# teofum/yart

Measured on NVIDIA B200. Metric: Mrays/s at 1080p (primary + shadow rays, reference ray count), higher is better.
Workload: dtype f32

## Files before the change

include/yart_cuda.h:

```cpp
#ifndef YART_CUDA_H
#define YART_CUDA_H

#include <stddef.h>
#include <stdint.h>

#ifdef __cplusplus
extern "C" {
#endif

#define YC_OK 0
#define YC_ERR_INVALID (-1)
#define YC_ERR_CUDA (-2)
#define YC_ERR_NO_SCENE (-3)
#define YC_ERR_NO_DEVICE (-4)
#define YC_ERR_STATE (-5)
#define YC_ERR_IO (-6)
#define YC_ERR_UNSUPPORTED (-7)

#define YC_ERR_ABORTED (-8)

#define YC_MAX_NODE_DEPTH 16


typedef struct YcNode {
// ... 171 lines not shown

typedef struct YcStats {
  uint64_t raysReference;
  uint64_t raysExtend;
  uint64_t raysShadow;
  uint64_t samples;
  uint64_t kernelLaunches;
  double gpuMs;
  uint64_t boxTests, triTests;
  double extendMs;
  uint64_t extendLaunches;
  double shadeMs;
  uint64_t shadeLaunches;
  uint64_t hitsShaded;
  double commMs;
} YcStats;

typedef struct YcRay { float o[3], tmin, d[3], tmax; } YcRay;

typedef struct YcHit {
  float t;
  uint32_t prim;
  int32_t material;
  int32_t lightIdx;
  uint32_t backSide;
  uint32_t didHit;
  float p[3], n[3], tg[3], uv[2];
  float attenuation[3];
} YcHit;

// ... 169 lines not shown
```

yart_b200/capi.py:

```python
from __future__ import annotations

import ctypes as C
import os

HERE = os.path.dirname(os.path.abspath(__file__))
PRODUCT_LIB = os.path.join(HERE, "libyart_b200.so")
SAMPLERS_LIB = os.path.join(HERE, "libyart_b200_samplers.so")

YC_OK, YC_ERR_INVALID, YC_ERR_CUDA, YC_ERR_NO_SCENE, YC_ERR_NO_DEVICE, YC_ERR_STATE, YC_ERR_IO = 0, -1, -2, -3, -4, -5, -6
YC_ERR_UNSUPPORTED = -7
TONEMAP_NONE, TONEMAP_AGX, TONEMAP_AGX_GOLDEN, TONEMAP_AGX_PUNCHY = 0, 1, 2, 3
ESTIMATOR_GMON, ESTIMATOR_MON, ESTIMATOR_MEAN, ESTIMATOR_GMONB = 0, 1, 2, 3
TRACE_CLOSEST, TRACE_ANY, TRACE_COUNT, TRACE_USE_TMAX, TRACE_REFERENCE_ORDER, TRACE_WIDE = 0, 1, 16, 32, 64, 128

f32, u32, i32, u64 = C.c_float, C.c_uint32, C.c_int32, C.c_uint64


class YcCamera(C.Structure):
    _fields_ = [("position", f32 * 3), ("topLeftPixel", f32 * 3), ("pixelDeltaU", f32 * 3), ("pixelDeltaV", f32 * 3),
                ("frameX", f32 * 3), ("frameY", f32 * 3), ("frameZ", f32 * 3), ("apertureRadius", f32),
                ("apertureSides", u32), ("exposure", f32)]


BVH_SAH, BVH_MEDIAN_SPLIT, BVH_SAH_DEVICE, BVH_SAH_HOST = 0, 1, 2, 3
# ... 11 lines not shown


class YcRect(C.Structure):
    _fields_ = [("x", u32), ("y", u32), ("w", u32), ("h", u32)]


class YcFrameDesc(C.Structure):
    _fields_ = [("width", u32), ("height", u32), ("totalSamples", u32), ("tileSize", u32), ("background", f32 * 3),
                ("tonemap", u32), ("estimator", u32), ("shardIndex", u32), ("shardCount", u32)]


class YcStats(C.Structure):
    _fields_ = [("raysReference", u64), ("raysExtend", u64), ("raysShadow", u64), ("samples", u64),
                ("kernelLaunches", u64), ("gpuMs", C.c_double), ("boxTests", u64), ("triTests", u64),
                ("extendMs", C.c_double), ("extendLaunches", u64), ("shadeMs", C.c_double), ("shadeLaunches", u64),
                ("hitsShaded", u64), ("commMs", C.c_double)]


class YcRay(C.Structure):
    _fields_ = [("o", f32 * 3), ("tmin", f32), ("d", f32 * 3), ("tmax", f32)]


class YcHit(C.Structure):
    _fields_ = [("t", f32), ("prim", u32), ("material", i32), ("lightIdx", i32), ("backSide", u32), ("didHit", u32),
                ("p", f32 * 3), ("n", f32 * 3), ("tg", f32 * 3), ("uv", f32 * 2), ("attenuation", f32 * 3)]


class YcMesh(C.Structure):
    _fields_ = [("rootMin", f32 * 3), ("rootMax", f32 * 3), ("rootRef", u32), ("nodeOffset", u32), ("triOffset", u32),
                ("vertOffset", u32), ("primOffset", u32), ("nTris", u32), ("nVerts", u32), ("nInner", u32)]

# ... 146 lines not shown
```

yart_b200/csrc/integrator.cuh:

```cuda
#pragma once
#include "camera.cuh"
#include "lights.cuh"
#include "wide_bvh.cuh"

namespace yb {

constexpr uint32_t kFlagDepthMask = 0xffu;
constexpr uint32_t kFlagSpecular = 1u << 8;
constexpr uint32_t kFlagRegularized = 1u << 9;
constexpr uint32_t kFlagPendingRR = 1u << 10;
constexpr int32_t kHitMiss = -1;
constexpr int32_t kHitDead = -2;
constexpr uint32_t kBackSideBit = 1u << 30;

struct PathState {
  float4* rayO;
  float4* rayD;
  float4* L;
  float4* att;
  uint32_t* dim;
  uint32_t* flags;
  float4* hitA;
  int32_t* hitB;
};
// ... 98 lines not shown
  st.hit.prim = 0xffffffffu;
  st.hit.node = kHitMiss;
  st.hit.backSide = 0;
  st.attenuation = V3(1.0f);
}

template <bool ALPHA, bool COUNT, bool WIDE = false>
YB_DEV void extendStage(const DScene& sc, const WaveParams& w, const PathState& ps, uint32_t i, TravStack& stack,
                        TraceCounters& cnt) {
  static_assert(!(ALPHA && WIDE), "the wide walk does not reproduce the order of alpha-test sampler draws");
  V3 o, d;
  Sampler smp;
  if (!extendLoad<ALPHA>(w, ps, i, o, d, smp)) return;
  TraceState st;
  initTraceState(st, INFINITY);
  if (WIDE) traceSceneWide<false, COUNT, false>(sc, o, d, st, stack, cnt);
  else traceScene<false, ALPHA, COUNT, false>(sc, o, d, st, stack, &smp, cnt);
  extendStore<ALPHA>(ps, i, st, smp);
}

struct ShadowRequest {
  V3 o, d, lif, att;
  float tMax, absDotN, denom;
};

enum : uint32_t { kShadeContinue = 1u, kShadeShadow = 2u };

YB_DEV void shadeMissStage(const DScene& sc, const WaveParams& w, const PathState& ps, uint32_t i, uint32_t& raysReference) {
  raysReference += 1;
  const float4 ro4 = ps.rayO[i], rd4 = ps.rayD[i], L4 = ps.L[i], a4 = ps.att[i];
  const V3 rayD(rd4.x, rd4.y, rd4.z);
// ... 280 lines not shown
  V3 L(L4.x, L4.y, L4.z);
  L += V3(a4.x, a4.y, a4.z) * Ld;
  ps.L[i] = make_float4(L.x, L.y, L.z, 0.0f);
  return 1u;
}

template <bool ALPHA, bool COUNT, bool WIDE = false>
YB_DEV uint32_t shadowStage(const DScene& sc, const WaveParams& w, const PathState& ps, const ShadowQueue& q,
                            uint32_t j, TravStack& stack, TraceCounters& cnt) {
  V3 o, d;
  float tMax;
  Sampler smp;
  const uint32_t i = shadowLoad<ALPHA>(w, ps, q, j, o, d, tMax, smp);
  TraceState st;
  initTraceState(st, tMax);
  const bool occluded = WIDE ? traceSceneWide<true, COUNT, true>(sc, o, d, st, stack, cnt)
                             : traceScene<true, ALPHA, COUNT, !ALPHA>(sc, o, d, st, stack, &smp, cnt);
  return shadowFinish<ALPHA>(ps, q, j, i, st, occluded, smp);
}

}
```

yart_b200/csrc/trace_kernels.cuh:

```cuda
#pragma once
#include "integrator.cuh"

namespace yb {

constexpr int kTraceBlock = 128;

struct TraceTuning {
  int refillMin;
  int innerMin;
  int shEntries;
};

constexpr int kPsStack = kShStack + 1;
constexpr uint32_t kPsStride = kTraceBlock * 8;
constexpr int kSpillEntries = kMaxStack;
struct WarpStack {
  uint32_t base;
  uint32_t limit;
  uint2** spillBase;
  __device__ __forceinline__ void init(uint2* shStack, uint2** shSpill, uint2* spill, int shEntries) {
    base = uint32_t(__cvta_generic_to_shared(shStack + threadIdx.x));
    const uint32_t l = base + uint32_t(shEntries) * kPsStride;
    asm volatile("mov.u32 %0, %1;" : "=r"(limit) : "r"(l));
    if (threadIdx.x == 0) *shSpill = spill;
// ... 13 lines not shown
    }
    if (on) sa += kPsStride;
  }
  __device__ __forceinline__ void popIf(bool on, uint32_t& sa, uint32_t& ref, float& d) const {
    if (on) sa -= kPsStride;
    uint32_t x = ref, y = __float_as_uint(d);
    if (on && sa < limit) asm volatile("ld.shared.v2.u32 {%0, %1}, [%2];" : "=r"(x), "=r"(y) : "r"(sa));
    if (on && sa >= limit) {
      const uint2 v = *spillSlot(spillBase, sa - limit);
      x = v.x, y = v.y;
    }
    ref = x;
    d = __uint_as_float(y);
  }
  __device__ __forceinline__ void pop(uint32_t& sa, uint32_t& ref, float& d) const { popIf(true, sa, ref, d); }
};

__device__ __forceinline__ void nodeLocalRay(const DScene& sc, uint32_t node, int depth, V3& o, V3& d) {
  const int32_t* __restrict__ path = sc.nodePath + size_t(node) * YC_MAX_NODE_DEPTH;
#pragma unroll 1
  for (int level = 0; level <= depth; level++) {
    const YcNode& nd = sc.nodes[path[level]];
    const V3 no = xformRows(nd.inv, o, 1.0f), ndir = xformRows(nd.inv, d, 0.0f);
    o = no;
    d = ndir;
  }
}

struct NodeRec {
  float f[16];
// ... 187 lines not shown
```

yart_b200/csrc/trace_wide.cuh:

```cuda
#pragma once
#include "trace_kernels.cuh"

namespace yb {

struct Words8 {
  uint32_t w[8];
};
__device__ __forceinline__ Words8 loadHalfNode(const float4* p) {
  Words8 r;
  asm volatile("ld.global.nc.v8.b32 {%0,%1,%2,%3,%4,%5,%6,%7}, [%8];"
               : "=r"(r.w[0]), "=r"(r.w[1]), "=r"(r.w[2]), "=r"(r.w[3]), "=r"(r.w[4]), "=r"(r.w[5]), "=r"(r.w[6]), "=r"(r.w[7])
               : "l"(p));
  return r;
}

template <bool NEE, bool COUNT, class IO>
__device__ __forceinline__ void traceWidePersistent(const DScene& sc, IO& io, uint32_t n, uint32_t* head, uint2* spillBase,
                                                    const TraceTuning tune, TraceCounters& cnt) {
  __shared__ uint2 shStack[kPsStack * kTraceBlock];
  __shared__ uint2* shSpill;
  WarpStack stack;
  stack.init(shStack, &shSpill, spillBase, tune.shEntries);
  const unsigned FULL = 0xffffffffu;
  const unsigned lane = threadIdx.x & 31u, ltMask = (1u << lane) - 1u;

  int state = kLaneIdle;
  bool exhausted = false;
  uint32_t item = 0, nextNode = 0, cur = 0;
  uint32_t sp = 0;
  int curNode = 0;
  float dcur = 0.0f;
// ... 131 lines not shown
        } else {
          stack.pushIf(q0, sp, rf.x, t0);
          stack.pushIf(q1, sp, rf.y, t1);
          stack.pushIf(q2, sp, rf.z, t2);
          stack.pushIf(q3, sp, rf.w, t3);
        }
        cur = any ? nearRef : kPopRef;
        dcur = best;
      }
    }

    if (state == kLaneTrav && (int32_t(cur) < 0 || pend != 0u)) {
      {
        const uint32_t leaf = pend;
        const float leafD = pendD;
        if (int32_t(leaf) < -3 && leafD < st.hit.t && !(NEE && didHit)) {
          const YcMesh& mesh = sc.meshes[meshIdx];
          uint32_t ti = leaf & ~YC_REF_LEAF;
          while (true) {
            const float4 a = __ldg(tris + 3 * size_t(ti)), b = __ldg(tris + 3 * size_t(ti) + 1),
                         c = __ldg(tris + 3 * size_t(ti) + 2);
            meshHit |= testTriangle<NEE, false, COUNT>(sc, mesh, r, a, b, c, curNode, st, &smp, cnt);
            if (NEE && meshHit) break;
            if (__float_as_uint(c.z) & YC_TRI_LAST) break;
            ti++;
          }
          didHit |= meshHit;
        }
      }
      pend = 0u;
      if (NEE && didHit) {
        io.store(item, st, true, smp);
        state = kLaneIdle;
      } else if (cur == kNoRef) {
        state = kLaneNode;
      }
    }
  }
}

}
```

yart_b200/csrc/wavefront.cu:

```cuda
#include <algorithm>
#include <cstdarg>
#include <vector>

#include "estimator.cuh"
#include "integrator.cuh"
#include "rt.cuh"
#include "comm.cuh"
#include "bvh_build.cuh"
#ifndef YB_HOSTSIM
#include "trace_wide.cuh"
#endif

using namespace yb;

#ifndef YB_TRACE_MIN_BLOCKS
#define YB_TRACE_MIN_BLOCKS 7
#endif
#ifndef YB_SHADOW_MIN_BLOCKS
#define YB_SHADOW_MIN_BLOCKS 7
#endif
#ifndef YB_RESOLVE_MIN_BLOCKS
#define YB_RESOLVE_MIN_BLOCKS 4
#endif
#ifndef YB_SAMPLE_MIN_BLOCKS
// ... 55 lines not shown
  size_t bucketCapacity = 0;
  bool bucketsDirty = false;

  uint32_t* dCtr = nullptr;
  void* dSpill = nullptr;
  Counters* dCounters = nullptr;
  std::vector<void*> waveAllocs;

  rt::Event ev0, ev1;
  bool wavesPending = false;
  rt::Event evFinal;
  std::vector<std::pair<rt::Event, rt::Event>> extendEvents;
  size_t extendEventsUsed = 0;
  std::vector<std::pair<rt::Event, rt::Event>> shadeEvents;
  size_t shadeEventsUsed = 0;
  double shadeMs = 0, commMs = 0;
  uint64_t shadeLaunches = 0, hitsShaded = 0;
  bool timeShade = false;
  bool oneLane = false;
  uint64_t launches = 0;
  double gpuMs = 0, extendMs = 0;
  uint64_t extendLaunches = 0, raysExtend = 0;
  bool timeExtend = false, countTraversal = false;
  uint32_t tailThreshold = 16384;
  const volatile int32_t* abortFlag = nullptr;
  std::unique_ptr<Comm> comm;
  bool wide = false;
  int wideDepth = 0;
  uint64_t nWideNodes = 0;
};

static int settleWaves(yc_ctx* ctx);

// ... 323 lines not shown
  if (COUNT) {
    aggregatedCount(&counters->boxTests, cnt.box);
    aggregatedCount(&counters->triTests, cnt.tri);
  }
}

#ifndef YB_WIDE_MIN_BLOCKS
#define YB_WIDE_MIN_BLOCKS 7
#endif
template <bool COUNT>
__global__ void __launch_bounds__(kTraceBlock, YB_WIDE_MIN_BLOCKS) extendWideKernel(DScene sc, WaveParams w, PathState ps, const uint32_t* queue,
                                                              uint32_t n, uint32_t* ctr, Counters* counters, uint2* spill,
                                                              TraceTuning tune) {
  ExtendIO<false> io{w, ps, queue};
  TraceCounters cnt;
  traceWidePersistent<false, COUNT>(sc, io, n, ctr + kCtrExtendHead, spill, tune, cnt);
  if (COUNT) {
    aggregatedCount(&counters->boxTests, cnt.box);
    aggregatedCount(&counters->triTests, cnt.tri);
  }
}

template <bool COUNT>
__global__ void __launch_bounds__(kTraceBlock, YB_WIDE_MIN_BLOCKS) shadowWideKernel(DScene sc, WaveParams w, PathState ps, ShadowQueue sq,
                                                              uint32_t* ctr, Counters* counters, uint2* spill, TraceTuning tune) {
  const uint32_t n = ctr[kCtrShadowCount];
  ShadowIO<false> io{w, ps, sq};
  TraceCounters cnt;
  traceWidePersistent<true, COUNT>(sc, io, n, ctr + kCtrShadowHead, spill, tune, cnt);
  aggregatedCount(&counters->raysReference, io.contributed);
  if (blockIdx.x == 0 && threadIdx.x == 0) atomicAdd(&counters->raysShadow, (unsigned long long)n);
  if (COUNT) {
    aggregatedCount(&counters->boxTests, cnt.box);
    aggregatedCount(&counters->triTests, cnt.tri);
  }
}

constexpr int kTailBlock = 128;
struct TailGatherK {
  PathState ps, ts;
  const uint32_t* queue;
  uint32_t* tq;
  YB_DEV void operator()(uint32_t j) const {
    const uint32_t i = queue[j];
// ... 89 lines not shown
      rt::eventCreate(ctx->extendEvents.back().second);
    }
    ev = &ctx->extendEvents[ctx->extendEventsUsed++];
    rt::eventRecord(L.st, ev->first);
  }
  if (!ALPHA && !COUNT && ctx->wide)
    extendWideKernel<false><<<traceGrid(ctx, n), kTraceBlock, 0, L.st.s>>>(ctx->ds, L.w, L.ps, L.qA, n, L.ctr, ctx->dCounters,
                                                                           static_cast<uint2*>(L.spill), tuning(ctx));
  else
    extendKernel<ALPHA, COUNT><<<traceGrid(ctx, n), kTraceBlock, 0, L.st.s>>>(ctx->ds, L.w, L.ps, L.qA, n, L.ctr, ctx->dCounters,
                                                                              static_cast<uint2*>(L.spill), tuning(ctx));
  if (ev) rt::eventRecord(L.st, ev->second);
}
template <bool ALPHA, bool COUNT>
static void runShadow(yc_ctx* ctx, Lane& L, uint32_t upperBound) {
  if (!ALPHA && !COUNT && ctx->wide)
    shadowWideKernel<false><<<traceGrid(ctx, upperBound), kTraceBlock, 0, L.st.s>>>(
      ctx->ds, L.w, L.ps, L.sq, L.ctr, ctx->dCounters, static_cast<uint2*>(L.spill), tuning(ctx));
  else
    shadowKernel<ALPHA, COUNT><<<traceGrid(ctx, upperBound), kTraceBlock, 0, L.st.s>>>(
      ctx->ds, L.w, L.ps, L.sq, L.ctr, ctx->dCounters, static_cast<uint2*>(L.spill), tuning(ctx));
}
#endif

extern "C" int yc_create(int device, const YcOptions* opts, yc_ctx** out) {
  if (!out) return YC_ERR_INVALID;
  *out = nullptr;
  yc_ctx* ctx = new (std::nothrow) yc_ctx();
  if (!ctx) return YC_ERR_INVALID;
  if (opts) ctx->opts = *opts;
  if (ctx->opts.maxDepth == 0) ctx->opts.maxDepth = 30;
  if (ctx->opts.integrator > YC_INTEGRATOR_NAIVE || ctx->opts.scrambler > YC_SCRAMBLER_BINARY_PERMUTE ||
      ctx->opts.sampler > YC_SAMPLER_STRATIFIED || ctx->opts.lightSampler > YC_LIGHT_SAMPLER_UNIFORM ||
      ctx->opts.traversal > YC_TRAVERSAL_WIDE ||
      (ctx->opts.integrator == YC_INTEGRATOR_NAIVE && ctx->opts.maxDepth + 1 > kNaiveMaxSegments)) {
    delete ctx;
// ... 54 lines not shown

static void destroyComm(yc_ctx* ctx);
static void detachCombinedFrames(yc_ctx* ctx);

extern "C" void yc_destroy(yc_ctx* ctx) {
  if (!ctx) return;
  enter(ctx);
  rt::sync(ctx->st);
  destroyComm(ctx);
  freeFrame(ctx);
  freeAll(ctx->sceneAllocs);
  freeAll(ctx->waveAllocs);
  rt::eventDestroy(ctx->ev0);
  rt::eventDestroy(ctx->ev1);
  rt::eventDestroy(ctx->evFinal);
  for (auto* evs : {&ctx->extendEvents, &ctx->shadeEvents})
    for (auto& ev : *evs) {
      rt::eventDestroy(ev.first);
      rt::eventDestroy(ev.second);
    }
  for (int l = 0; l < kLanes; l++) {
    Lane& L = ctx->lanes[l];
    rt::sync(L.st);
    rt::sync(L.side);
    rt::hostRelease(L.hCtr);
    rt::eventDestroy(L.evCtr);
    rt::eventDestroy(L.evChunk);
    rt::eventDestroy(L.evTail);
    rt::eventDestroy(L.evSide[0]);
    rt::eventDestroy(L.evSide[1]);
    rt::destroy(L.side);
// ... 246 lines not shown
      return fail(ctx, YC_ERR_CUDA, "yc_begin_frame: %s", e);
    }
    ctx->bucketsDirty = true;
  }
  ctx->frame = *f;
  ctx->frame.shardCount = shardCount;
  if (ctx->bucketsDirty) {
    YC_TRY(rt::zero(ctx->st, ctx->dBuckets, ctx->bucketCapacity * kMaxBuckets * sizeof(float4)));
    ctx->bucketsDirty = false;
  }
  YC_TRY(rt::zero(ctx->st, ctx->dHdr, frameTexels * sizeof(float4)));
  YC_TRY(rt::zero(ctx->st, ctx->dLdr, frameTexels * sizeof(float4)));
  YC_TRY(rt::zero(ctx->st, ctx->dCounters, sizeof(Counters)));
  YC_TRY(rt::sync(ctx->st));
  ctx->launches = 0;
  ctx->gpuMs = ctx->extendMs = ctx->shadeMs = ctx->commMs = 0;
  ctx->extendLaunches = ctx->shadeLaunches = ctx->hitsShaded = 0;
  ctx->raysExtend = 0;
  ctx->inFrame = true;
  return YC_OK;
}

template <bool ALPHA>
static int issueBounce(yc_ctx* ctx, Lane& L) {
  const uint32_t n = L.n;
  YC_TRY(rt::zero(L.st, L.ctr, kCtrCount * sizeof(uint32_t)));
  if (ctx->countTraversal) runExtend<ALPHA, true>(ctx, L, n);
  else runExtend<ALPHA, false>(ctx, L, n);
  rt::launchFor(L.st, n, SortMissK{ctx->ds, L.w, L.ps, L.qA, L.qH, L.ctr, ctx->dCounters});
  std::pair<rt::Event, rt::Event>* sev = nullptr;
  if (ctx->timeShade) {
    if (ctx->shadeEventsUsed == ctx->shadeEvents.size()) {
// ... 256 lines not shown
    YC_TRY(rt::sync(ctx->lanes[l].st));
    YC_TRY(rt::sync(ctx->lanes[l].side));
  }
  YC_TRY(rt::lastError());
  ctx->gpuMs += rt::eventElapsedMs(ctx->ev0, ctx->ev1);
  for (size_t i = 0; i < ctx->extendEventsUsed; i++) {
    ctx->extendMs += rt::eventElapsedMs(ctx->extendEvents[i].first, ctx->extendEvents[i].second);
    ctx->extendLaunches++;
  }
  ctx->extendEventsUsed = 0;
  for (size_t i = 0; i < ctx->shadeEventsUsed; i++) {
    ctx->shadeMs += rt::eventElapsedMs(ctx->shadeEvents[i].first, ctx->shadeEvents[i].second);
    ctx->shadeLaunches++;
  }
  ctx->shadeEventsUsed = 0;
  return YC_OK;
}

static int accumulateWave(yc_ctx* ctx, const uint32_t* dList, uint32_t nPixCall, uint32_t sampleOffset, uint32_t waveSamples,
                          uint32_t bucketShard, uint32_t bucketShardCount) {
  const uint32_t m = waveBuckets(ctx->frame, waveSamples);
  ctx->bucketsDirty = true;
  return ctx->ds.hasAlpha ? renderChunks<true>(ctx, dList, nPixCall, sampleOffset, waveSamples, m, bucketShard, bucketShardCount)
                          : renderChunks<false>(ctx, dList, nPixCall, sampleOffset, waveSamples, m, bucketShard, bucketShardCount);
}

static void finalizeWave(yc_ctx* ctx, const uint32_t* dList, uint32_t nPixCall, uint32_t waveSamples, uint32_t takenBefore) {
  const YcFrameDesc& f = ctx->frame;
  const uint32_t takenAfter = takenBefore + waveSamples;
  const float wCurrent = float(takenBefore) / float(takenAfter), wWave = float(waveSamples) / float(takenAfter);
// ... 113 lines not shown
  if (!stats) return YC_OK;
  Counters c{};
  if (ctx->dCounters) YC_TRY(rt::d2h(ctx->st, &c, ctx->dCounters, sizeof c));
  memset(stats, 0, sizeof *stats);
  stats->raysReference = c.raysReference;
  stats->raysExtend = ctx->raysExtend + c.raysExtend;
  stats->raysShadow = c.raysShadow;
  stats->boxTests = c.boxTests;
  stats->triTests = c.triTests;
  stats->kernelLaunches = ctx->launches;
  stats->gpuMs = ctx->gpuMs;
  stats->extendMs = ctx->extendMs;
  stats->shadeMs = ctx->shadeMs, stats->shadeLaunches = ctx->shadeLaunches, stats->hitsShaded = ctx->hitsShaded;
  stats->commMs = ctx->commMs;
  stats->extendLaunches = ctx->extendLaunches;
  return YC_OK;
}

extern "C" int yc_resolve(yc_ctx* ctx, float* hdrRGBA, float* ldrRGBA, YcStats* stats) {
  if (!ctx) return YC_ERR_INVALID;
  YC_ENTER(ctx);
  if (!ctx->inFrame) return fail(ctx, YC_ERR_STATE, "yc_resolve before yc_begin_frame");
  const size_t bytes = size_t(ctx->frame.width) * ctx->frame.height * sizeof(float4);
  if (hdrRGBA) YC_TRY(rt::d2h(ctx->st, hdrRGBA, ctx->dHdr, bytes));
  if (ldrRGBA) YC_TRY(rt::d2h(ctx->st, ldrRGBA, ctx->dLdr, bytes));
  return readStats(ctx, stats);
}

extern "C" int yc_frame_device_ptrs(yc_ctx* ctx, void** hdr, void** ldr, size_t* bytes) {
  if (!ctx) return YC_ERR_INVALID;
// ... 11 lines not shown
  if (!ctx->inFrame) return fail(ctx, YC_ERR_STATE, "no frame");
  rt::launchFor(ctx->st, ctx->frame.width * ctx->frame.height, RetonemapK{ctx->dHdr, ctx->dLdr, ctx->frame.tonemap});
  ctx->launches++;
  YC_TRY(rt::sync(ctx->st));
  YC_TRY(rt::lastError());
  return YC_OK;
}

extern "C" int yc_set_profiling(yc_ctx* ctx, int timeExtendKernel) {
  if (!ctx) return YC_ERR_INVALID;
  YC_ENTER(ctx);
  ctx->timeExtend = (timeExtendKernel & 1) != 0;
  ctx->countTraversal = (timeExtendKernel & 2) != 0;
  ctx->timeShade = (timeExtendKernel & 4) != 0;
  ctx->oneLane = (timeExtendKernel & 8) != 0;
  return YC_OK;
}

YB_DEV Sampler traceHookSampler() {
  SamplerConfig c;
  c.log2spp = 4;
  c.nBase4Digits = 6 + 2;
  c.scrambler = kScrambleFastOwen;
  c.kind = kSamplerSobol;
  c.strata = 4;
  Sampler s;
  s.start(c, 0, 0, 0);
  return s;
}

template <bool NEE, bool ALPHA, bool COUNT, bool WIDE = false>
YB_DEV void traceOne(const DScene& sc, const YcRay& ray, bool useTMax, YcHit& out, TravStack& stack, TraceCounters& cnt) {
  Sampler smp = traceHookSampler();
  TraceState st;
  st.hit.t = (NEE || useTMax) ? ray.tmax : INFINITY;
  st.hit.node = kHitMiss;
  st.hit.u = st.hit.v = 0.0f;
  st.hit.prim = 0xffffffffu;
  st.hit.backSide = 0;
  st.attenuation = V3(1.0f);
  const V3 o(ray.o), d(ray.d);
  const bool did = WIDE ? traceSceneWide<NEE, COUNT, NEE>(sc, o, d, st, stack, cnt)
                        : traceScene<NEE, ALPHA, COUNT, false>(sc, o, d, st, stack, &smp, cnt);
  out.t = st.hit.t;
  out.didHit = did ? 1u : 0u;
  out.prim = did ? st.hit.prim : 0xffffffffu;
  out.material = -1, out.lightIdx = -1, out.backSide = 0;
  for (int k = 0; k < 3; k++) out.p[k] = out.n[k] = out.tg[k] = 0.0f;
  out.uv[0] = out.uv[1] = 0.0f;
  out.attenuation[0] = st.attenuation.x, out.attenuation[1] = st.attenuation.y, out.attenuation[2] = st.attenuation.z;
  if (did) {
    const SurfaceHit s = resolveHit(sc, st.hit, o, d);
    out.material = s.material, out.lightIdx = s.lightIdx, out.backSide = st.hit.backSide;
    out.p[0] = s.p.x, out.p[1] = s.p.y, out.p[2] = s.p.z;
    out.n[0] = s.n.x, out.n[1] = s.n.y, out.n[2] = s.n.z;
    out.tg[0] = s.tg.x, out.tg[1] = s.tg.y, out.tg[2] = s.tg.z;
    out.uv[0] = s.uv.x, out.uv[1] = s.uv.y;
// ... 74 lines not shown
  TraceIO<NEE, ALPHA, COMPACT> io{sc, rays, hits, compact, useTMax};
  TraceCounters cnt;
  tracePersistent<NEE, ALPHA, COUNT, false>(sc, io, n, head, spill, tune, cnt);
  if (COUNT) {
    aggregatedCount(&counters->boxTests, cnt.box);
    aggregatedCount(&counters->triTests, cnt.tri);
  }
}

template <bool NEE, bool COUNT, bool COMPACT>
__global__ void __launch_bounds__(kTraceBlock, YB_WIDE_MIN_BLOCKS) traceWideKernel(DScene sc, const YcRay* rays, uint32_t n, int useTMax, YcHit* hits,
                                                             CompactHit* compact, uint32_t* head, Counters* counters,
                                                             uint2* spill, TraceTuning tune) {
  TraceIO<NEE, false, COMPACT> io{sc, rays, hits, compact, useTMax};
  TraceCounters cnt;
  traceWidePersistent<NEE, COUNT>(sc, io, n, head, spill, tune, cnt);
  if (COUNT) {
    aggregatedCount(&counters->boxTests, cnt.box);
    aggregatedCount(&counters->triTests, cnt.tri);
  }
}

template <bool NEE, bool ALPHA, bool COUNT, bool WIDE = false>
static void runTrace(yc_ctx* ctx, const YcRay* rays, uint32_t n, bool useTMax, YcHit* hits, CompactHit* compact) {
  const int grid = traceGrid(ctx, n);
  uint2* spill = static_cast<uint2*>(ctx->dSpill);
  if (WIDE) {
    if (compact)
      traceWideKernel<NEE, COUNT, true><<<grid, kTraceBlock, 0, ctx->st.s>>>(ctx->ds, rays, n, useTMax, hits, compact, ctx->dCtr,
                                                                             ctx->dCounters, spill, tuning(ctx));
    else
// ... 587 lines not shown
```

yart_b200/csrc/wide_bvh.cuh:

```cuda
#pragma once
#include <vector>

#include "traverse.cuh"

#include <atomic>
#include <chrono>
#include <cstdio>
#include <cstdlib>
#include <thread>

namespace yb {

constexpr uint32_t kWideEmpty = 0xfffffffdu;

struct WideNode {
  float pS[3];
  float S[3];
  uint32_t q[6];
  uint32_t ref[4];
};
static_assert(sizeof(WideNode) == 64, "WideNode is two 32-byte sectors");

struct WideChildBox {
  float lo[3], hi[3];
// ... 212 lines not shown
  return tn <= tf;
}

template <int K>
YB_DEV float planeUnit(uint32_t word, uint32_t one) {
#ifdef YB_HOSTSIM
  return __uint_as_float(__byte_perm(word, one, 0x7604u | (uint32_t(K) << 4)));
#else
  uint32_t r;
  asm("prmt.b32 %0, %1, %2, %3;" : "=r"(r) : "r"(word), "r"(one), "n"(0x7604 | (K << 4)));
  return __uint_as_float(r);
#endif
}

struct WideSlabs {
  float tn[4];
  bool hit[4];
};
template <int K>
YB_DEV void slabWideChild(WideSlabs& r, uint32_t one, uint32_t nx, uint32_t ny, uint32_t nz, uint32_t fx, uint32_t fy, uint32_t fz,
                          float Sx, float Sy, float Sz, float Bx, float By, float Bz, float tmn, float tmx, bool live) {
  const float tnx = fmaExact(planeUnit<K>(nx, one), Sx, Bx), tny = fmaExact(planeUnit<K>(ny, one), Sy, By),
              tnz = fmaExact(planeUnit<K>(nz, one), Sz, Bz);
  const float tfx = fmaExact(planeUnit<K>(fx, one), Sx, Bx), tfy = fmaExact(planeUnit<K>(fy, one), Sy, By),
              tfz = fmaExact(planeUnit<K>(fz, one), Sz, Bz);
  r.tn[K] = fmaxf(fmaxf(tnx, tny), fmaxf(tnz, tmn));
  const float tf = fminf(fminf(tfx, tfy), fminf(tfz, tmx));
  r.hit[K] = live && r.tn[K] <= tf;
}
YB_DEV WideSlabs slabWide4(const WideRay& w, uint32_t one, float px, float py, float pz, float sx, float sy, float sz, uint32_t qlx,
                           uint32_t qhx, uint32_t qly, uint32_t qhy, uint32_t qlz, uint32_t qhz, float tmn, float tmx, bool live) {
  const float Sx = sx * w.idir.x, Sy = sy * w.idir.y, Sz = sz * w.idir.z;
  const float Bx = fmaExact(px, w.idir.x, w.odir.x), By = fmaExact(py, w.idir.y, w.odir.y), Bz = fmaExact(pz, w.idir.z, w.odir.z);
  const uint32_t nx = (qlx & ~w.mx) | (qhx & w.mx), fx = (qhx & ~w.mx) | (qlx & w.mx);
  const uint32_t ny = (qly & ~w.my) | (qhy & w.my), fy = (qhy & ~w.my) | (qly & w.my);
  const uint32_t nz = (qlz & ~w.mz) | (qhz & w.mz), fz = (qhz & ~w.mz) | (qlz & w.mz);
  WideSlabs r;
  slabWideChild<0>(r, one, nx, ny, nz, fx, fy, fz, Sx, Sy, Sz, Bx, By, Bz, tmn, tmx, live);
  slabWideChild<1>(r, one, nx, ny, nz, fx, fy, fz, Sx, Sy, Sz, Bx, By, Bz, tmn, tmx, live);
  slabWideChild<2>(r, one, nx, ny, nz, fx, fy, fz, Sx, Sy, Sz, Bx, By, Bz, tmn, tmx, live);
  slabWideChild<3>(r, one, nx, ny, nz, fx, fy, fz, Sx, Sy, Sz, Bx, By, Bz, tmn, tmx, live);
  return r;
}

template <bool NEE, bool COUNT, bool EARLY_OUT>
YB_DEV bool testBVHWide(const DScene& sc, const YcMesh& mesh, const WideMesh& wm, const LocalRay& r, const WideRay& w,
                        int nodeIdx, TraceState& st, TravStack& stack, TraceCounters& cnt) {
  float d;
  if (COUNT) cnt.box++;
  if (!slabWideBox(w, V3(mesh.rootMin), V3(mesh.rootMax), kTMin, st.hit.t, d)) return false;
  const float4* __restrict__ nodes = sc.wideNodes + 4 * size_t(wm.nodeOffset);
  const float4* __restrict__ tris = sc.bvhTris + 3 * size_t(mesh.triOffset);
  uint32_t cur = wm.rootRef;
  int sp = 0;
  bool didHit = false;
  while (true) {
    if (d < st.hit.t) {
      if (cur & YC_REF_LEAF) {
        uint32_t ti = cur & ~YC_REF_LEAF;
        while (true) {
          const float4 a = __ldg(tris + 3 * size_t(ti)), b = __ldg(tris + 3 * size_t(ti) + 1),
                       c = __ldg(tris + 3 * size_t(ti) + 2);
          didHit |= testTriangle<NEE, false, COUNT>(sc, mesh, r, a, b, c, nodeIdx, st, nullptr, cnt);
          if (NEE && didHit) break;
          if (__float_as_uint(c.z) & YC_TRI_LAST) break;
          ti++;
        }
        if (NEE && EARLY_OUT && didHit) return true;
        if (sp == 0) break;
        stack.pop(--sp, cur, d);
      } else {
        const float4* n = nodes + 4 * size_t(cur);
        const float4 r0 = __ldg(n), r1 = __ldg(n + 1), r2 = __ldg(n + 2), rf = __ldg(n + 3);
        const uint32_t ref[4] = {__float_as_uint(rf.x), __float_as_uint(rf.y), __float_as_uint(rf.z), __float_as_uint(rf.w)};
        WideSlabs sl = slabWide4(w, 0x3f800000u, r0.x, r0.y, r0.z, r0.w, r1.x, r1.y, __float_as_uint(r1.z), __float_as_uint(r1.w),
                                 __float_as_uint(r2.x), __float_as_uint(r2.y), __float_as_uint(r2.z), __float_as_uint(r2.w), kTMin,
                                 st.hit.t, true);
        float* tn = sl.tn;
        bool* hit = sl.hit;
        hit[2] = hit[2] && ref[2] != kWideEmpty;
        hit[3] = hit[3] && ref[3] != kWideEmpty;
        if (COUNT) cnt.box += 2u + (ref[2] != kWideEmpty) + (ref[3] != kWideEmpty);
        int nearSlot = -1;
// ... 5 lines not shown
        } else {
          for (int k = 0; k < 4; k++)
            if (hit[k] && k != nearSlot) stack.push(sp++, ref[k], tn[k]);
          cur = ref[nearSlot];
          d = tn[nearSlot];
        }
      }
    } else {
      if (sp == 0) break;
      stack.pop(--sp, cur, d);
    }
  }
  return didHit;
}

template <bool NEE, bool COUNT, bool EARLY_OUT>
YB_DEV bool traceSceneWide(const DScene& sc, V3 origin, V3 dir, TraceState& st, TravStack& stack, TraceCounters& cnt) {
  V3 ro[YC_MAX_NODE_DEPTH + 1], rd[YC_MAX_NODE_DEPTH + 1];
  ro[0] = origin;
  rd[0] = dir;
  bool didHit = false;
  uint32_t i = 0;
  while (i < sc.nNodes) {
    const YcNode& nd = sc.nodes[i];
    const int k = nd.depth;
    LocalRay r;
    r.o = xformRows(nd.inv, ro[k], 1.0f), r.d = xformRows(nd.inv, rd[k], 0.0f);
    ro[k + 1] = r.o;
    rd[k + 1] = r.d;
    WideRay w;
    w.set(r.o, r.d);
    float d;
    if (COUNT) cnt.box++;
    if (!slabWideBox(w, V3(nd.bmin), V3(nd.bmax), kTMin, st.hit.t, d) || st.hit.t < d) {
      i = uint32_t(nd.skip);
      continue;
    }
    if (nd.mesh >= 0) {
      const bool h = testBVHWide<NEE, COUNT, EARLY_OUT>(sc, sc.meshes[nd.mesh], sc.wideMeshes[nd.mesh], r, w, int(i), st, stack, cnt);
      didHit |= h;
      if (NEE && EARLY_OUT && h) return true;
    }
    i++;
  }
  return didHit;
}

}
```

yart_b200/host/api.cpp:

```cpp
#include <atomic>
#include <chrono>
#include <mutex>
#include <new>
#include <thread>
#include <cstring>
#include <vector>

#include "scene.hpp"

using namespace yartb;

namespace yartb {
bool loadGlb(const std::string& path, ysc::SceneDesc& out, std::string* err);
bool writePpm(const std::string& path, const float* rgba, uint32_t w, uint32_t h);
bool decodeTextureForTest(const uint8_t* png, size_t len, uint32_t type, int C, const int* channels, ysc::TextureDesc& out,
                          std::string& err);
bool decodeRadianceHdr(const uint8_t* data, size_t len, int& w, int& h, std::vector<float>& rgb, std::string& err);
}

struct ys_scene {
  HostScene host;
};

static thread_local std::string g_ysError;
// ... 568 lines not shown
  return writePpm(path, ldr.data(), r->s.width, r->s.height) ? YC_OK : rfail(r, YC_ERR_IO, std::string("cannot write ") + path);
}

extern "C" int yr_read(yr_renderer* r, float* hdrRGBA, float* ldrRGBA, YcStats* stats) {
  if (!r) return YC_ERR_INVALID;
  int rc = readFrames(r, hdrRGBA, ldrRGBA);
  if (rc != YC_OK) return rfail(r, rc, yc_last_error(r->shards[0].ctx));
  if (stats) {
    memset(stats, 0, sizeof *stats);
    for (Shard& sh : r->shards) {
      YcStats st{};
      if ((rc = yc_resolve(sh.ctx, nullptr, nullptr, &st)) != YC_OK) return rfail(r, rc, yc_last_error(sh.ctx));
      stats->raysReference += st.raysReference, stats->raysExtend += st.raysExtend, stats->raysShadow += st.raysShadow;
      stats->kernelLaunches += st.kernelLaunches, stats->boxTests += st.boxTests, stats->triTests += st.triTests;
      stats->gpuMs = std::max(stats->gpuMs, st.gpuMs), stats->extendMs += st.extendMs, stats->extendLaunches += st.extendLaunches;
    }
  }
  return YC_OK;
}

extern "C" const float* ys_lut_tables(size_t* count) {
  static HostScene holder;
  static std::once_flag once;
  std::call_once(once, [] {
    std::string err;
    holder.loadLuts(&err);
  });
  if (count) *count = holder.lutTables.size();
  return holder.lutTables.empty() ? nullptr : holder.lutTables.data();
}
// ... 1 lines not shown
```

Before: 1073.

## Add dedicated any-hit wide BVH traversal for shadow rays with ref-only stack

Splits shadow/any-hit traversal out of the closest-hit persistent wide BVH walker into its own kernel path. The new path keeps a 32-bit ref-only shared stack with no distances, and orders children by slab overlap length instead of entry distance so likely occluders are visited first. It also returns on the first triangle hit. The aim is to cut shared-memory traffic, register pressure and wasted node visits for occlusion rays. In exchange it adds code duplication plus some shadow-kernel timing instrumentation, and the child-ordering heuristic may not pay off on every scene.

```diff
diff --git a/include/yart_cuda.h b/include/yart_cuda.h
--- a/include/yart_cuda.h
+++ b/include/yart_cuda.h
@@ -209,6 +209,8 @@
   uint64_t shadeLaunches;
   uint64_t hitsShaded;
   double commMs;
+  double shadowMs;
+  uint64_t shadowLaunches;
 } YcStats;
 
 typedef struct YcRay { float o[3], tmin, d[3], tmax; } YcRay;
diff --git a/yart_b200/capi.py b/yart_b200/capi.py
--- a/yart_b200/capi.py
+++ b/yart_b200/capi.py
@@ -49,7 +49,7 @@
     _fields_ = [("raysReference", u64), ("raysExtend", u64), ("raysShadow", u64), ("samples", u64),
                 ("kernelLaunches", u64), ("gpuMs", C.c_double), ("boxTests", u64), ("triTests", u64),
                 ("extendMs", C.c_double), ("extendLaunches", u64), ("shadeMs", C.c_double), ("shadeLaunches", u64),
-                ("hitsShaded", u64), ("commMs", C.c_double)]
+                ("hitsShaded", u64), ("commMs", C.c_double), ("shadowMs", C.c_double), ("shadowLaunches", u64)]
 
 
 class YcRay(C.Structure):
diff --git a/yart_b200/csrc/integrator.cuh b/yart_b200/csrc/integrator.cuh
--- a/yart_b200/csrc/integrator.cuh
+++ b/yart_b200/csrc/integrator.cuh
@@ -136,7 +136,7 @@
   if (!extendLoad<ALPHA>(w, ps, i, o, d, smp)) return;
   TraceState st;
   initTraceState(st, INFINITY);
-  if (WIDE) traceSceneWide<false, COUNT, false>(sc, o, d, st, stack, cnt);
+  if (WIDE) traceSceneWide<false, COUNT>(sc, o, d, st, stack, cnt);
   else traceScene<false, ALPHA, COUNT, false>(sc, o, d, st, stack, &smp, cnt);
   extendStore<ALPHA>(ps, i, st, smp);
 }
@@ -447,7 +447,7 @@
   const uint32_t i = shadowLoad<ALPHA>(w, ps, q, j, o, d, tMax, smp);
   TraceState st;
   initTraceState(st, tMax);
-  const bool occluded = WIDE ? traceSceneWide<true, COUNT, true>(sc, o, d, st, stack, cnt)
+  const bool occluded = WIDE ? traceSceneWide<true, COUNT>(sc, o, d, st, stack, cnt)
                              : traceScene<true, ALPHA, COUNT, !ALPHA>(sc, o, d, st, stack, &smp, cnt);
   return shadowFinish<ALPHA>(ps, q, j, i, st, occluded, smp);
 }
diff --git a/yart_b200/csrc/trace_kernels.cuh b/yart_b200/csrc/trace_kernels.cuh
--- a/yart_b200/csrc/trace_kernels.cuh
+++ b/yart_b200/csrc/trace_kernels.cuh
@@ -51,6 +51,38 @@
     d = __uint_as_float(y);
   }
   __device__ __forceinline__ void pop(uint32_t& sa, uint32_t& ref, float& d) const { popIf(true, sa, ref, d); }
+};
+
+constexpr uint32_t kRsStride = kTraceBlock * 4;
+struct WarpRefStack {
+  uint32_t base, limit;
+  uint2** spillBase;
+  __device__ __forceinline__ void init(uint32_t* shStack, uint2** shSpill, uint2* spill, int shEntries) {
+    base = uint32_t(__cvta_generic_to_shared(shStack + threadIdx.x));
+    const uint32_t l = base + uint32_t(shEntries) * kRsStride;
+    asm volatile("mov.u32 %0, %1;" : "=r"(limit) : "r"(l));
+    if (threadIdx.x == 0) *shSpill = spill;
+    __syncthreads();
+    spillBase = shSpill;
+  }
+  __device__ __noinline__ static uint32_t* spillSlot(uint2** spillBase, uint32_t off) {
+    return reinterpret_cast<uint32_t*>(*spillBase + size_t(blockIdx.x * kTraceBlock + threadIdx.x) * kSpillEntries) + off / kRsStride;
+  }
+  __device__ __forceinline__ void put(uint32_t sa, uint32_t ref) const { asm volatile("st.shared.u32 [%0], %1;" ::"r"(sa), "r"(ref)); }
+  __device__ __forceinline__ void pushIf(bool on, uint32_t& sa, uint32_t ref) const {
+    if (on && sa < limit) put(sa, ref);
+    if (on && sa >= limit) {
+      if (sa < base + uint32_t(kMaxStack + 1) * kRsStride) *spillSlot(spillBase, sa - limit) = ref;
+    }
+    if (on) sa += kRsStride;
+  }
+  __device__ __forceinline__ void popIf(bool on, uint32_t& sa, uint32_t& ref) const {
+    if (on) sa -= kRsStride;
+    uint32_t x = ref;
+    if (on && sa < limit) asm volatile("ld.shared.u32 %0, [%1];" : "=r"(x) : "r"(sa));
+    if (on && sa >= limit) x = *spillSlot(spillBase, sa - limit);
+    ref = x;
+  }
 };
 
 __device__ __forceinline__ void nodeLocalRay(const DScene& sc, uint32_t node, int depth, V3& o, V3& d) {
diff --git a/yart_b200/csrc/trace_wide.cuh b/yart_b200/csrc/trace_wide.cuh
--- a/yart_b200/csrc/trace_wide.cuh
+++ b/yart_b200/csrc/trace_wide.cuh
@@ -14,7 +14,7 @@
   return r;
 }
 
-template <bool NEE, bool COUNT, class IO>
+template <bool COUNT, class IO>
 __device__ __forceinline__ void traceWidePersistent(const DScene& sc, IO& io, uint32_t n, uint32_t* head, uint2* spillBase,
                                                     const TraceTuning tune, TraceCounters& cnt) {
   __shared__ uint2 shStack[kPsStack * kTraceBlock];
@@ -176,14 +176,13 @@
       {
         const uint32_t leaf = pend;
         const float leafD = pendD;
-        if (int32_t(leaf) < -3 && leafD < st.hit.t && !(NEE && didHit)) {
+        if (int32_t(leaf) < -3 && leafD < st.hit.t) {
           const YcMesh& mesh = sc.meshes[meshIdx];
           uint32_t ti = leaf & ~YC_REF_LEAF;
           while (true) {
             const float4 a = __ldg(tris + 3 * size_t(ti)), b = __ldg(tris + 3 * size_t(ti) + 1),
                          c = __ldg(tris + 3 * size_t(ti) + 2);
-            meshHit |= testTriangle<NEE, false, COUNT>(sc, mesh, r, a, b, c, curNode, st, &smp, cnt);
-            if (NEE && meshHit) break;
+            meshHit |= testTriangle<false, false, COUNT>(sc, mesh, r, a, b, c, curNode, st, &smp, cnt);
             if (__float_as_uint(c.z) & YC_TRI_LAST) break;
             ti++;
           }
@@ -191,7 +190,175 @@
         }
       }
       pend = 0u;
-      if (NEE && didHit) {
+      if (cur == kNoRef) state = kLaneNode;
+    }
+  }
+}
+
+template <bool COUNT, class IO>
+__device__ __forceinline__ void anyHitWidePersistent(const DScene& sc, IO& io, uint32_t n, uint32_t* head, uint2* spillBase,
+                                                     const TraceTuning tune, TraceCounters& cnt) {
+  __shared__ uint32_t shStack[kPsStack * kTraceBlock];
+  __shared__ uint2* shSpill;
+  WarpRefStack stack;
+  stack.init(shStack, &shSpill, spillBase, tune.shEntries);
+  const unsigned FULL = 0xffffffffu;
+  const unsigned lane = threadIdx.x & 31u, ltMask = (1u << lane) - 1u;
+
+  int state = kLaneIdle;
+  bool exhausted = false;
+  uint32_t item = 0, nextNode = 0, cur = 0;
+  uint32_t sp = 0;
+  int curNode = 0;
+  bool rayIsWorld = false, worldFinite = false;
+  V3 wo, wd;
+  LocalRay r;
+  WideRay wr;
+  TraceState st;
+  Sampler smp;
+  const float4* __restrict__ nodes = nullptr;
+  const float4* __restrict__ tris = nullptr;
+  uint32_t meshIdx = 0;
+  constexpr uint32_t kNoRef = 0xffffffffu;
+  constexpr uint32_t kPopRef = 0xfffffffeu;
+  uint32_t pend = 0u;
+  const uint32_t one = 0x3f800000u | (uint32_t(tune.shEntries) >> 30);
+
+  for (;;) {
+    const unsigned idle = __ballot_sync(FULL, state == kLaneIdle);
+    if (idle) {
+      if (!exhausted && (__popc(idle) >= tune.refillMin || idle == FULL)) {
+        const uint32_t want = uint32_t(__popc(idle));
+        uint32_t base = 0;
+        if (lane == 0) base = atomicAdd(head, want);
+        base = __shfl_sync(FULL, base, 0);
+        if (state == kLaneIdle) {
+          const uint32_t j = base + uint32_t(__popc(idle & ltMask));
+          if (j < n) {
+            float tMax;
+            if (io.load(j, wo, wd, tMax, smp)) {
+              item = j;
+              rayIsWorld = false;
+              worldFinite = isfinite(wo.x) && isfinite(wo.y) && isfinite(wo.z) && isfinite(wd.x) && isfinite(wd.y) &&
+                            isfinite(wd.z);
+              initTraceState(st, tMax);
+              nextNode = 0;
+              state = kLaneNode;
+            }
+          }
+        }
+        if (base + want >= n) exhausted = true;
+      }
+      if (exhausted && __ballot_sync(FULL, state != kLaneIdle) == 0) break;
+    }
+
+    if (state == kLaneNode) {
+      bool entered = false;
+      while (nextNode < sc.nNodes) {
+        const YcNode& nd = sc.nodes[nextNode];
+        if (nd.identityChain && worldFinite) {
+          if (!rayIsWorld) {
+            r.o = wo + 0.0f, r.d = wd + 0.0f;
+            wr.set(r.o, r.d);
+            rayIsWorld = true;
+          }
+        } else {
+          V3 o = wo, d = wd;
+          nodeLocalRay(sc, nextNode, nd.depth, o, d);
+          r.o = o, r.d = d;
+          wr.set(o, d);
+          rayIsWorld = false;
+        }
+        float dd;
+        if (COUNT) cnt.box++;
+        if (!slabWideBox(wr, V3(nd.bmin), V3(nd.bmax), kTMin, st.hit.t, dd) || st.hit.t < dd) {
+          nextNode = uint32_t(nd.skip);
+          continue;
+        }
+        const int mi = nd.mesh;
+        curNode = int(nextNode);
+        nextNode++;
+        if (mi < 0) continue;
+        const YcMesh& mesh = sc.meshes[mi];
+        if (COUNT) cnt.box++;
+        if (!slabWideBox(wr, V3(mesh.rootMin), V3(mesh.rootMax), kTMin, st.hit.t, dd)) continue;
+        const WideMesh wm = sc.wideMeshes[mi];
+        meshIdx = uint32_t(mi);
+        nodes = sc.wideNodes + 4 * size_t(wm.nodeOffset);
+        tris = sc.bvhTris + 3 * size_t(mesh.triOffset);
+        cur = wm.rootRef;
+        stack.put(stack.base, kNoRef);
+        sp = stack.base + kRsStride;
+        pend = 0u;
+        entered = true;
+        break;
+      }
+      if (entered) {
+        state = kLaneTrav;
+      } else {
+        io.store(item, st, false, smp);
+        state = kLaneIdle;
+      }
+    }
+
+    for (;;) {
+      const bool trav = state == kLaneTrav;
+#ifdef YB_X_NOPARK
+      bool doPop = trav && cur == kPopRef && pend == 0u;
+      if (trav && pend == 0u && int32_t(cur) < -3) {
+        pend = cur;
+        cur = kPopRef;
+      }
+#else
+      bool doPop = trav && cur == kPopRef;
+      if (trav && pend == 0u && int32_t(cur) < -3) {
+        pend = cur;
+        doPop = true;
+      }
+#endif
+      stack.popIf(doPop, sp, cur);
+      const bool inner = trav && int32_t(cur) >= 0;
+      const unsigned im = __ballot_sync(FULL, inner);
+      if (im == 0) break;
+      if (__popc(im) < tune.innerMin && __ballot_sync(FULL, trav && !inner)) break;
+      if (inner) {
+        const float4* np = nodes + 4 * size_t(cur);
+        const Words8 a = loadHalfNode(np), b = loadHalfNode(np + 2);
+        uint32_t rf[4] = {b.w[4], b.w[5], b.w[6], b.w[7]};
+        const WideSlabs sl = slabWide4(wr, one, __uint_as_float(a.w[0]), __uint_as_float(a.w[1]), __uint_as_float(a.w[2]),
+                                       __uint_as_float(a.w[3]), __uint_as_float(a.w[4]), __uint_as_float(a.w[5]), a.w[6], a.w[7], b.w[0],
+                                       b.w[1], b.w[2], b.w[3], kTMin, st.hit.t, true);
+        if (COUNT) cnt.box += 2u + (rf[2] != kWideEmpty) + (rf[3] != kWideEmpty);
+        float k[4];
+        anyHitChildOrder(sl, sl.hit[0], sl.hit[1], sl.hit[2] && rf[2] != kWideEmpty, sl.hit[3] && rf[3] != kWideEmpty, k, rf);
+        const bool q1 = k[1] < INFINITY, q2 = k[2] < INFINITY, q3 = k[3] < INFINITY;
+        if (sp + 3u * kRsStride < stack.limit) {
+          uint32_t sa = sp;
+          if (q3) stack.put(sa, rf[3]), sa += kRsStride;
+          if (q2) stack.put(sa, rf[2]), sa += kRsStride;
+          if (q1) stack.put(sa, rf[1]), sa += kRsStride;
+          sp = sa;
+        } else {
+          stack.pushIf(q3, sp, rf[3]);
+          stack.pushIf(q2, sp, rf[2]);
+          stack.pushIf(q1, sp, rf[1]);
+        }
+        cur = k[0] < INFINITY ? rf[0] : kPopRef;
+      }
+    }
+
+    if (state == kLaneTrav && (int32_t(cur) < 0 || pend != 0u)) {
+      bool hit = false;
+      if (int32_t(pend) < -3) {
+        const YcMesh& mesh = sc.meshes[meshIdx];
+        for (uint32_t ti = pend & ~YC_REF_LEAF;; ti++) {
+          const float4 a = __ldg(tris + 3 * size_t(ti)), b = __ldg(tris + 3 * size_t(ti) + 1), c = __ldg(tris + 3 * size_t(ti) + 2);
+          hit = testTriangle<true, false, COUNT>(sc, mesh, r, a, b, c, curNode, st, &smp, cnt);
+          if (hit || (__float_as_uint(c.z) & YC_TRI_LAST)) break;
+        }
+      }
+      pend = 0u;
+      if (hit) {
         io.store(item, st, true, smp);
         state = kLaneIdle;
       } else if (cur == kNoRef) {
diff --git a/yart_b200/csrc/wavefront.cu b/yart_b200/csrc/wavefront.cu
--- a/yart_b200/csrc/wavefront.cu
+++ b/yart_b200/csrc/wavefront.cu
@@ -93,9 +93,11 @@
   size_t extendEventsUsed = 0;
   std::vector<std::pair<rt::Event, rt::Event>> shadeEvents;
   size_t shadeEventsUsed = 0;
-  double shadeMs = 0, commMs = 0;
-  uint64_t shadeLaunches = 0, hitsShaded = 0;
-  bool timeShade = false;
+  std::vector<std::pair<rt::Event, rt::Event>> shadowEvents;
+  size_t shadowEventsUsed = 0;
+  double shadeMs = 0, commMs = 0, shadowMs = 0;
+  uint64_t shadeLaunches = 0, hitsShaded = 0, shadowLaunches = 0;
+  bool timeShade = false, timeShadow = false;
   bool oneLane = false;
   uint64_t launches = 0;
   double gpuMs = 0, extendMs = 0;
@@ -449,7 +451,7 @@
                                                               TraceTuning tune) {
   ExtendIO<false> io{w, ps, queue};
   TraceCounters cnt;
-  traceWidePersistent<false, COUNT>(sc, io, n, ctr + kCtrExtendHead, spill, tune, cnt);
+  traceWidePersistent<COUNT>(sc, io, n, ctr + kCtrExtendHead, spill, tune, cnt);
   if (COUNT) {
     aggregatedCount(&counters->boxTests, cnt.box);
     aggregatedCount(&counters->triTests, cnt.tri);
@@ -457,12 +459,15 @@
 }
 
 template <bool COUNT>
-__global__ void __launch_bounds__(kTraceBlock, YB_WIDE_MIN_BLOCKS) shadowWideKernel(DScene sc, WaveParams w, PathState ps, ShadowQueue sq,
+#ifndef YB_X_SHADOW_BLOCKS
+#define YB_X_SHADOW_BLOCKS YB_WIDE_MIN_BLOCKS
+#endif
+__global__ void __launch_bounds__(kTraceBlock, YB_X_SHADOW_BLOCKS) shadowWideKernel(DScene sc, WaveParams w, PathState ps, ShadowQueue sq,
                                                               uint32_t* ctr, Counters* counters, uint2* spill, TraceTuning tune) {
   const uint32_t n = ctr[kCtrShadowCount];
   ShadowIO<false> io{w, ps, sq};
   TraceCounters cnt;
-  traceWidePersistent<true, COUNT>(sc, io, n, ctr + kCtrShadowHead, spill, tune, cnt);
+  anyHitWidePersistent<COUNT>(sc, io, n, ctr + kCtrShadowHead, spill, tune, cnt);
   aggregatedCount(&counters->raysReference, io.contributed);
   if (blockIdx.x == 0 && threadIdx.x == 0) atomicAdd(&counters->raysShadow, (unsigned long long)n);
   if (COUNT) {
@@ -582,12 +587,23 @@
 }
 template <bool ALPHA, bool COUNT>
 static void runShadow(yc_ctx* ctx, Lane& L, uint32_t upperBound) {
+  std::pair<rt::Event, rt::Event>* ev = nullptr;
+  if (ctx->timeShadow) {
+    if (ctx->shadowEventsUsed == ctx->shadowEvents.size()) {
+      ctx->shadowEvents.emplace_back();
+      rt::eventCreate(ctx->shadowEvents.back().first);
+      rt::eventCreate(ctx->shadowEvents.back().second);
+    }
+    ev = &ctx->shadowEvents[ctx->shadowEventsUsed++];
+    rt::eventRecord(L.st, ev->first);
+  }
   if (!ALPHA && !COUNT && ctx->wide)
     shadowWideKernel<false><<<traceGrid(ctx, upperBound), kTraceBlock, 0, L.st.s>>>(
       ctx->ds, L.w, L.ps, L.sq, L.ctr, ctx->dCounters, static_cast<uint2*>(L.spill), tuning(ctx));
   else
     shadowKernel<ALPHA, COUNT><<<traceGrid(ctx, upperBound), kTraceBlock, 0, L.st.s>>>(
       ctx->ds, L.w, L.ps, L.sq, L.ctr, ctx->dCounters, static_cast<uint2*>(L.spill), tuning(ctx));
+  if (ev) rt::eventRecord(L.st, ev->second);
 }
 #endif
 
@@ -672,7 +688,7 @@
   rt::eventDestroy(ctx->ev0);
   rt::eventDestroy(ctx->ev1);
   rt::eventDestroy(ctx->evFinal);
-  for (auto* evs : {&ctx->extendEvents, &ctx->shadeEvents})
+  for (auto* evs : {&ctx->extendEvents, &ctx->shadeEvents, &ctx->shadowEvents})
     for (auto& ev : *evs) {
       rt::eventDestroy(ev.first);
       rt::eventDestroy(ev.second);
@@ -949,8 +965,8 @@
   YC_TRY(rt::zero(ctx->st, ctx->dCounters, sizeof(Counters)));
   YC_TRY(rt::sync(ctx->st));
   ctx->launches = 0;
-  ctx->gpuMs = ctx->extendMs = ctx->shadeMs = ctx->commMs = 0;
-  ctx->extendLaunches = ctx->shadeLaunches = ctx->hitsShaded = 0;
+  ctx->gpuMs = ctx->extendMs = ctx->shadeMs = ctx->commMs = ctx->shadowMs = 0;
+  ctx->extendLaunches = ctx->shadeLaunches = ctx->hitsShaded = ctx->shadowLaunches = 0;
   ctx->raysExtend = 0;
   ctx->inFrame = true;
   return YC_OK;
@@ -1237,6 +1253,11 @@
     ctx->shadeLaunches++;
   }
   ctx->shadeEventsUsed = 0;
+  for (size_t i = 0; i < ctx->shadowEventsUsed; i++) {
+    ctx->shadowMs += rt::eventElapsedMs(ctx->shadowEvents[i].first, ctx->shadowEvents[i].second);
+    ctx->shadowLaunches++;
+  }
+  ctx->shadowEventsUsed = 0;
   return YC_OK;
 }
 
@@ -1380,6 +1401,7 @@
   stats->shadeMs = ctx->shadeMs, stats->shadeLaunches = ctx->shadeLaunches, stats->hitsShaded = ctx->hitsShaded;
   stats->commMs = ctx->commMs;
   stats->extendLaunches = ctx->extendLaunches;
+  stats->shadowMs = ctx->shadowMs, stats->shadowLaunches = ctx->shadowLaunches;
   return YC_OK;
 }
 
@@ -1421,6 +1443,7 @@
   ctx->countTraversal = (timeExtendKernel & 2) != 0;
   ctx->timeShade = (timeExtendKernel & 4) != 0;
   ctx->oneLane = (timeExtendKernel & 8) != 0;
+  ctx->timeShadow = (timeExtendKernel & 16) != 0;
   return YC_OK;
 }
 
@@ -1447,7 +1470,7 @@
   st.hit.backSide = 0;
   st.attenuation = V3(1.0f);
   const V3 o(ray.o), d(ray.d);
-  const bool did = WIDE ? traceSceneWide<NEE, COUNT, NEE>(sc, o, d, st, stack, cnt)
+  const bool did = WIDE ? traceSceneWide<NEE, COUNT>(sc, o, d, st, stack, cnt)
                         : traceScene<NEE, ALPHA, COUNT, false>(sc, o, d, st, stack, &smp, cnt);
   out.t = st.hit.t;
   out.didHit = did ? 1u : 0u;
@@ -1552,7 +1575,8 @@
                                                              uint2* spill, TraceTuning tune) {
   TraceIO<NEE, false, COMPACT> io{sc, rays, hits, compact, useTMax};
   TraceCounters cnt;
-  traceWidePersistent<NEE, COUNT>(sc, io, n, head, spill, tune, cnt);
+  if (NEE) anyHitWidePersistent<COUNT>(sc, io, n, head, spill, tune, cnt);
+  else traceWidePersistent<COUNT>(sc, io, n, head, spill, tune, cnt);
   if (COUNT) {
     aggregatedCount(&counters->boxTests, cnt.box);
     aggregatedCount(&counters->triTests, cnt.tri);
diff --git a/yart_b200/csrc/wide_bvh.cuh b/yart_b200/csrc/wide_bvh.cuh
--- a/yart_b200/csrc/wide_bvh.cuh
+++ b/yart_b200/csrc/wide_bvh.cuh
@@ -250,7 +250,7 @@
 }
 
 struct WideSlabs {
-  float tn[4];
+  float tn[4], tf[4];
   bool hit[4];
 };
 template <int K>
@@ -261,8 +261,8 @@
   const float tfx = fmaExact(planeUnit<K>(fx, one), Sx, Bx), tfy = fmaExact(planeUnit<K>(fy, one), Sy, By),
               tfz = fmaExact(planeUnit<K>(fz, one), Sz, Bz);
   r.tn[K] = fmaxf(fmaxf(tnx, tny), fmaxf(tnz, tmn));
-  const float tf = fminf(fminf(tfx, tfy), fminf(tfz, tmx));
-  r.hit[K] = live && r.tn[K] <= tf;
+  r.tf[K] = fminf(fminf(tfx, tfy), fminf(tfz, tmx));
+  r.hit[K] = live && r.tn[K] <= r.tf[K];
 }
 YB_DEV WideSlabs slabWide4(const WideRay& w, uint32_t one, float px, float py, float pz, float sx, float sy, float sz, uint32_t qlx,
                            uint32_t qhx, uint32_t qly, uint32_t qhy, uint32_t qlz, uint32_t qhz, float tmn, float tmx, bool live) {
@@ -279,7 +279,27 @@
   return r;
 }
 
-template <bool NEE, bool COUNT, bool EARLY_OUT>
+YB_DEV void anyHitExchange(float& ka, uint32_t& ra, float& kb, uint32_t& rb) {
+  const bool s = kb < ka;
+  const float lo = s ? kb : ka, hi = s ? ka : kb;
+  const uint32_t rl = s ? rb : ra, rh = s ? ra : rb;
+  ka = lo, kb = hi, ra = rl, rb = rh;
+}
+YB_DEV void anyHitChildOrder(const WideSlabs& sl, bool h0, bool h1, bool h2, bool h3, float k[4], uint32_t r[4]) {
+#ifdef YB_X_NEAREST
+  k[0] = h0 ? sl.tn[0] : INFINITY, k[1] = h1 ? sl.tn[1] : INFINITY, k[2] = h2 ? sl.tn[2] : INFINITY, k[3] = h3 ? sl.tn[3] : INFINITY;
+#else
+  k[0] = h0 ? fminf(sl.tn[0] - sl.tf[0], 0.0f) : INFINITY, k[1] = h1 ? fminf(sl.tn[1] - sl.tf[1], 0.0f) : INFINITY;
+  k[2] = h2 ? fminf(sl.tn[2] - sl.tf[2], 0.0f) : INFINITY, k[3] = h3 ? fminf(sl.tn[3] - sl.tf[3], 0.0f) : INFINITY;
+#endif
+  anyHitExchange(k[0], r[0], k[1], r[1]);
+  anyHitExchange(k[2], r[2], k[3], r[3]);
+  anyHitExchange(k[0], r[0], k[2], r[2]);
+  anyHitExchange(k[1], r[1], k[3], r[3]);
+  anyHitExchange(k[1], r[1], k[2], r[2]);
+}
+
+template <bool COUNT>
 YB_DEV bool testBVHWide(const DScene& sc, const YcMesh& mesh, const WideMesh& wm, const LocalRay& r, const WideRay& w,
                         int nodeIdx, TraceState& st, TravStack& stack, TraceCounters& cnt) {
   float d;
@@ -297,12 +317,10 @@
         while (true) {
           const float4 a = __ldg(tris + 3 * size_t(ti)), b = __ldg(tris + 3 * size_t(ti) + 1),
                        c = __ldg(tris + 3 * size_t(ti) + 2);
-          didHit |= testTriangle<NEE, false, COUNT>(sc, mesh, r, a, b, c, nodeIdx, st, nullptr, cnt);
-          if (NEE && didHit) break;
+          didHit |= testTriangle<false, false, COUNT>(sc, mesh, r, a, b, c, nodeIdx, st, nullptr, cnt);
           if (__float_as_uint(c.z) & YC_TRI_LAST) break;
           ti++;
         }
-        if (NEE && EARLY_OUT && didHit) return true;
         if (sp == 0) break;
         stack.pop(--sp, cur, d);
       } else {
@@ -338,7 +356,46 @@
   return didHit;
 }
 
-template <bool NEE, bool COUNT, bool EARLY_OUT>
+template <bool COUNT>
+YB_DEV bool anyHitBVHWide(const DScene& sc, const YcMesh& mesh, const WideMesh& wm, const LocalRay& r, const WideRay& w,
+                          int nodeIdx, TraceState& st, TravStack& stack, TraceCounters& cnt) {
+  float d;
+  if (COUNT) cnt.box++;
+  if (!slabWideBox(w, V3(mesh.rootMin), V3(mesh.rootMax), kTMin, st.hit.t, d)) return false;
+  const float4* __restrict__ nodes = sc.wideNodes + 4 * size_t(wm.nodeOffset);
+  const float4* __restrict__ tris = sc.bvhTris + 3 * size_t(mesh.triOffset);
+  uint32_t cur = wm.rootRef;
+  int sp = 0;
+  while (true) {
+    if (cur & YC_REF_LEAF) {
+      for (uint32_t ti = cur & ~YC_REF_LEAF;; ti++) {
+        const float4 a = __ldg(tris + 3 * size_t(ti)), b = __ldg(tris + 3 * size_t(ti) + 1), c = __ldg(tris + 3 * size_t(ti) + 2);
+        if (testTriangle<true, false, COUNT>(sc, mesh, r, a, b, c, nodeIdx, st, nullptr, cnt)) return true;
+        if (__float_as_uint(c.z) & YC_TRI_LAST) break;
+      }
+    } else {
+      const float4* n = nodes + 4 * size_t(cur);
+      const float4 r0 = __ldg(n), r1 = __ldg(n + 1), r2 = __ldg(n + 2), rf = __ldg(n + 3);
+      uint32_t ref[4] = {__float_as_uint(rf.x), __float_as_uint(rf.y), __float_as_uint(rf.z), __float_as_uint(rf.w)};
+      const WideSlabs sl = slabWide4(w, 0x3f800000u, r0.x, r0.y, r0.z, r0.w, r1.x, r1.y, __float_as_uint(r1.z), __float_as_uint(r1.w),
+                                     __float_as_uint(r2.x), __float_as_uint(r2.y), __float_as_uint(r2.z), __float_as_uint(r2.w), kTMin,
+                                     st.hit.t, true);
+      if (COUNT) cnt.box += 2u + (ref[2] != kWideEmpty) + (ref[3] != kWideEmpty);
+      float k[4];
+      anyHitChildOrder(sl, sl.hit[0], sl.hit[1], sl.hit[2] && ref[2] != kWideEmpty, sl.hit[3] && ref[3] != kWideEmpty, k, ref);
+      if (k[0] < INFINITY) {
+        for (int i = 3; i >= 1; i--)
+          if (k[i] < INFINITY) stack.push(sp++, ref[i], 0.0f);
+        cur = ref[0];
+        continue;
+      }
+    }
+    if (sp == 0) return false;
+    stack.pop(--sp, cur, d);
+  }
+}
+
+template <bool NEE, bool COUNT>
 YB_DEV bool traceSceneWide(const DScene& sc, V3 origin, V3 dir, TraceState& st, TravStack& stack, TraceCounters& cnt) {
   V3 ro[YC_MAX_NODE_DEPTH + 1], rd[YC_MAX_NODE_DEPTH + 1];
   ro[0] = origin;
@@ -361,9 +418,10 @@
       continue;
     }
     if (nd.mesh >= 0) {
-      const bool h = testBVHWide<NEE, COUNT, EARLY_OUT>(sc, sc.meshes[nd.mesh], sc.wideMeshes[nd.mesh], r, w, int(i), st, stack, cnt);
+      const bool h = NEE ? anyHitBVHWide<COUNT>(sc, sc.meshes[nd.mesh], sc.wideMeshes[nd.mesh], r, w, int(i), st, stack, cnt)
+                         : testBVHWide<COUNT>(sc, sc.meshes[nd.mesh], sc.wideMeshes[nd.mesh], r, w, int(i), st, stack, cnt);
       didHit |= h;
-      if (NEE && EARLY_OUT && h) return true;
+      if (NEE && h) return true;
     }
     i++;
   }
diff --git a/yart_b200/host/api.cpp b/yart_b200/host/api.cpp
--- a/yart_b200/host/api.cpp
+++ b/yart_b200/host/api.cpp
@@ -606,6 +606,7 @@
       stats->raysReference += st.raysReference, stats->raysExtend += st.raysExtend, stats->raysShadow += st.raysShadow;
       stats->kernelLaunches += st.kernelLaunches, stats->boxTests += st.boxTests, stats->triTests += st.triTests;
       stats->gpuMs = std::max(stats->gpuMs, st.gpuMs), stats->extendMs += st.extendMs, stats->extendLaunches += st.extendLaunches;
+      stats->shadowMs += st.shadowMs, stats->shadowLaunches += st.shadowLaunches;
     }
   }
   return YC_OK;
```

New measurement: 1099 (median of 6 runs). 1.02x the previous value.
